# adi-gov-tw/Taiwan-Tongues-ASR-CE

Measured on AMD Instinct MI355X. Metric: audio-sec/s (RTF) whisper-large-v3 greedy, 30 s clips, batch 32; 1/2/4/8 GPU, higher is better.
Workload: dtype bf16; 1 GPU; whisper-large-v3 geometry (random-init seeded weights), 32 x 30 s 16 kHz synthetic clips per GPU in pinned host memory, H2D + log-mel + encoder + cross-KV + 4-token prompt + 128 greedy tokens (EOT suppressed), bf16; clips_per_gpu=32, contexts_per_gpu=1, parallelism=dp1

## Files before the change

taiwan_tongues_asr_ce_amd/csrc/common.hpp:

```cpp
#pragma once
#include <hip/hip_runtime.h>
#include <stdint.h>

typedef uint16_t bf16_t;

using f32x4 = __attribute__((ext_vector_type(4))) float;
using f32x16 = __attribute__((ext_vector_type(16))) float;
using s16x8 = __attribute__((ext_vector_type(8))) short;
using s16x4 = __attribute__((ext_vector_type(4))) short;

__device__ __forceinline__ float bf2f(bf16_t v) { return __uint_as_float(((uint32_t)v) << 16); }
__device__ __forceinline__ bf16_t f2bf(float f) { return __builtin_bit_cast(bf16_t, (__bf16)f); }
__device__ __forceinline__ uint32_t f2bf_pk(float lo, float hi) {
  typedef __bf16 bf16x2_hw __attribute__((ext_vector_type(2)));
  typedef float f32x2_hw __attribute__((ext_vector_type(2)));
  return __builtin_bit_cast(uint32_t, __builtin_convertvector((f32x2_hw){lo, hi}, bf16x2_hw));
}
struct f16_t { uint16_t bits; };
using h16x8 = __attribute__((ext_vector_type(8))) _Float16;
typedef _Float16 h16x2_hw __attribute__((ext_vector_type(2)));

template <typename T> struct N16;
template <> struct N16<bf16_t> {
  static __device__ __forceinline__ float up(uint16_t b) { return __uint_as_float(((uint32_t)b) << 16); }
// ... 90 lines not shown
  return v;
}
template <class T> __device__ __forceinline__ T* sgpr_pin_ptr(T* p) {
  typedef __attribute__((address_space(1))) T* global_ptr;
  global_ptr g = (global_ptr)p;
  asm volatile("" : "+s"(g));
  return (T*)g;
}


__device__ __forceinline__ int32_t sload_i32(const int32_t* p) {
  typedef const __attribute__((address_space(4))) int32_t* const_ptr;
  return *(const_ptr)p;
}
__device__ __forceinline__ int row_done_issue(const int32_t* done, int row, const void* valid) {
  return sload_i32(done ? done + row : (const int32_t*)valid);
}

struct GemmEpi {
  const float* bias = nullptr;
  int act = 0;
  const float* rowtab = nullptr;
  int rowmod = 0;
  const float* residual = nullptr;
  float* out_f32 = nullptr;
  void* out_t = nullptr;
  int64_t ldc = 0;
  int64_t batch_stride_c = 0;
  int headsplit = 0;
  int hs_T = 0, hs_H = 0, hs_d = 0;
  int64_t hs_which = 0;
};

struct GemmArgs {
  const void* A = nullptr;
  const void* W = nullptr;
  int M = 0, N = 0, K = 0;
  int64_t lda = 0, ldw = 0;
  int64_t batch_stride_a = 0;
  int batch = 1;
  int groups = 1;
  int64_t group_stride_w = 0, group_stride_out = 0;
  GemmEpi epi;
};

struct KernelOpts {
  int xattn_variant = 3;
  int xattn_deep_items = 512;
  int xattn_mq_slices = 0;
  int skinny_nt = 1;
  int skinny_narrow = 1;
  int skinny_x_lds = 1;
  int flash_qw = 2;
};

template <typename T> void launch_gemm_basic(const GemmArgs& g, hipStream_t s);
template <typename T16> void launch_gemm_bf16_fast(const GemmArgs& g, hipStream_t s);
bool gemm_bf16_fast_ok(const GemmArgs& g);
template <typename T16> void launch_gemm_bf16_v2(const GemmArgs& g, hipStream_t s);
bool gemm_bf16_v2_ok(const GemmArgs& g);
template <typename T16> void launch_gemm_bf16_v3(const GemmArgs& g, hipStream_t s);
bool gemm_bf16_v3_ok(const GemmArgs& g);
template <typename T16> void launch_gemm_bf16_v4(const GemmArgs& g, hipStream_t s);
bool gemm_bf16_v4_ok(const GemmArgs& g);
template <typename T16> bool launch_gemm_bf16_v5(const GemmArgs& g, hipStream_t s);
bool gemm_bf16_v5_ok(const GemmArgs& g);

template <typename T>
void launch_layernorm(const float* x, const float* gamma, const float* beta, T* out, int rows, int d, hipStream_t s);
template <typename T>
void launch_layernorm_add(float* x, const T* delta, const float* gamma, const float* beta, T* out, int rows, int d, hipStream_t s);
template <typename T>
void launch_layernorm_peek(const float* x, const T* delta, const float* gamma, const float* beta, T* out, int rows, int d, hipStream_t s);
template <typename T>
void launch_layernorm_add2(float* x, const T* delta, const T* delta2, const float* gamma, const float* beta, T* out, int rows, int d,
                           hipStream_t s);
struct LnPre {
  const float* bias = nullptr;
  const float* slab = nullptr;
  int n_slab = 0;
  int64_t slab_stride = 0;
  float* x_out = nullptr;
  const int32_t* tok = nullptr;
  const int32_t* step = nullptr;
  const void* emb = nullptr;
  const void* pos = nullptr;
};
template <typename T>
void launch_layernorm_rows(const float* x, const float* gamma, const float* beta, T* out, int rows, int d, const LnPre& pre,
                           hipStream_t s);
template <typename T>
void launch_layernorm_rows_embed_pos(const float* gamma, const float* beta, T* out, int rows, int d, const LnPre& pre, hipStream_t s);

struct SlabIn {
  const float* slab = nullptr;
  const float* bias = nullptr;
  int n = 0;
  int64_t stride = 0;
  int ld = 0;
};

template <typename T> struct RowVec;
template <> struct RowVec<float> {
  static constexpr int VEC = 4;
  __device__ static void load(const float* p, float (&v)[4]) {
    float4 t = *(const float4*)p;
// ... 2 lines not shown
};
template <typename T16> struct RowVec16 {
  static constexpr int VEC = 8;
  __device__ static void load(const T16* p, float (&v)[8]) {
    const uint4 t = *(const uint4*)p;
    up8<T16>(t, v);
  }
};
template <> struct RowVec<bf16_t> : RowVec16<bf16_t> {};
template <> struct RowVec<f16_t> : RowVec16<f16_t> {};

template <typename T>
__device__ __forceinline__ void load_row_slabs(const SlabIn& si, int64_t off, int col ,
                                               float (&v)[RowVec<T>::VEC]) {
  constexpr int VEC = RowVec<T>::VEC, NF4 = VEC / 4, MAXS = 4;
  float4 t[MAXS][NF4], bs[NF4];
#pragma unroll
  for (int c = 0; c < NF4; ++c) bs[c] = *(const float4*)(si.bias + col + 4 * c);
#pragma unroll
  for (int s = 0; s < MAXS; ++s) {
    const float* p = si.slab + (int64_t)min(s, si.n - 1) * si.stride + off;
#pragma unroll
    for (int c = 0; c < NF4; ++c) t[s][c] = *(const float4*)(p + 4 * c);
  }
  __builtin_amdgcn_sched_barrier(0);
#pragma unroll
  for (int c = 0; c < NF4; ++c) {
    float4 a = bs[c];
#pragma unroll
    for (int s = 0; s < MAXS; ++s)
      if (s == 0 || s < si.n) { a.x += t[s][c].x; a.y += t[s][c].y; a.z += t[s][c].z; a.w += t[s][c].w; }
    v[4 * c] = to_f<T>(from_f<T>(a.x)); v[4 * c + 1] = to_f<T>(from_f<T>(a.y));
    v[4 * c + 2] = to_f<T>(from_f<T>(a.z)); v[4 * c + 3] = to_f<T>(from_f<T>(a.w));
  }
}
struct QProj {
  const void* x = nullptr;
  const void* W = nullptr;
  const float* bias = nullptr;
};

template <typename T16> void launch_shuffle_cast(const float* src, T16* dst_base, int rows, int K, int row_offset, const KernelOpts& ko, hipStream_t s, int rows_total = 0);
int skinny_rows_per_block(int N, int K, const KernelOpts& ko);
template <typename T16>
bool launch_gemm_skinny(const T16* Wsh, const T16* x, int B, int N, int K, const GemmEpi& e, const KernelOpts& ko, hipStream_t s, int ksplit = 1,
                        float* slab = nullptr, int64_t slab_stride = 0);
int gemm_skinny_ksplit(int B, int N, int K, int want, const KernelOpts& ko);
template <typename T16> bool launch_gemm_vocab(const T16* Wsh, const T16* x, int B, int N, int K, float* out, int64_t ldc, const KernelOpts& ko, hipStream_t s, int device);
void gemm_vocab_init(int device);
void gemm_tiles_init(int device);
void launch_mel(const float* pcm, int64_t pcm_stride, const int64_t* n_samples_dev, int B, int n_mels, int n_frames,
                const float* filters , const float* dft_cos, const float* dft_sin ,
                const float* window , float* logmel , unsigned* clip_max ,
                hipStream_t s, const int64_t* geom_dev = nullptr);
unsigned mel_max_to_ordered(float v);
float mel_max_from_ordered(unsigned u);
template <typename T>
void launch_mel_finish(float* logmel, const unsigned* clip_max, T* mel_t , int B, int n_mels,
                       int n_frames, hipStream_t s, const int64_t* geom_dev = nullptr);
template <typename T>
void launch_mel_transpose(const float* mel, T* mel_t, int B, int n_mels, int n_frames, hipStream_t s);

template <typename T> void launch_enc_attn_simple(const T* qkv, T* out, int B, int T_, int H, hipStream_t s);
template <typename T16> void launch_enc_attn_flash_bf16(const T16* qkv, T16* out, int B, int T_, int H, const KernelOpts& ko, hipStream_t s);
template <typename T16>
void launch_cross_attn_flash_bf16(const T16* q, const T16* K, const T16* V, T16* out, int n_clips, int n_q, int H, int Tk, hipStream_t s);

struct RuleDyn { int32_t max_prompt, max_new, sot_index; uint32_t seed; };
struct DecState {
  int32_t* cur_tok;
  int32_t* step;
  int32_t* n_sampled;
  int32_t* last_tok;
  int32_t* pen_tok;
  int32_t* last_ts;
  int32_t* done;
  int32_t* n_done;
  float* sum_logprob;
  float* no_speech;
  int32_t* out_tokens;
  const int32_t* prompt;
  const int32_t* prompt_len;
  const uint8_t* mask;
  const RuleDyn* dyn;
  const int32_t* row_cap;
};
struct RuleParams {
  int V, ldv, max_prompt, max_new;
  int eot, no_timestamps, timestamp_begin, no_speech, sot_index, timestamps, max_initial, suppress_eot;
  float temperature;
  uint32_t seed;
};
template <typename T>
void launch_cross_attn_probs(const T* q, const T* K, const T* V, T* out, int rows, int H, int Tk, const int* sel ,
                             float* probs , hipStream_t s);
void launch_token_logprob(const float* logits, int ldv, int V, const int32_t* target, float* out, int rows, hipStream_t s);
void launch_token_prob(const float* logits, int ldv, int V, int tok, float* out , int rows, hipStream_t s);
template <typename T>
void launch_lang_head(const T* dh, const T* emb, int rows, int d, int V, int lang_begin, int n_lang, float* probs, int32_t* best,
                      float* logits, hipStream_t s);
struct LangRows {
  int32_t* pending; const int32_t* slot; int32_t* prompt; int max_prompt; int32_t* cur_tok; int32_t* row_pos;
  int32_t* best; float* probs; float* logits;
};
template <typename T>
void launch_lang_head_rows(const T* dh, const T* emb, int rows, int d, int V, int lang_begin, int n_lang, const LangRows& a, hipStream_t s);
void launch_lang_admit_rows(const int32_t* tab, int n, int B, int sot, int32_t* pending, int32_t* slot, int32_t* cur_tok, hipStream_t s);
// ... 74 lines not shown
```

taiwan_tongues_asr_ce_amd/csrc/engine.hip:

```cpp
#include "engine_ctx.hpp"
extern "C" {

const char* ttasr_version(void) { return "ttasr 0.4 (gfx950, HIP; f32 | bf16 | fp16)"; }

const char* ttasr_last_error(const ttasr_ctx* ctx) { return ctx ? ctx->err.c_str() : g_create_error.c_str(); }

static int create_impl(const ttasr_config* cfg, int device_id, ttasr_ctx* owner, ttasr_ctx** out_ctx);
static std::mutex g_share_mu;

int ttasr_create(const ttasr_config* cfg, int device_id, ttasr_ctx** out_ctx) {
  return guarded(nullptr, [&]() -> int { return create_impl(cfg, device_id, nullptr, out_ctx); });
}

int ttasr_create_shared(ttasr_ctx* owner, int32_t max_batch, ttasr_ctx** out_ctx) {
  return guarded(nullptr, [&]() -> int {
  if (!owner || !out_ctx) return fail(nullptr, TTASR_E_INVALID, "owner/out_ctx is NULL");
  *out_ctx = nullptr;
  if (owner->weight_owner) owner = owner->weight_owner;
  if (!owner->finalized) return fail(nullptr, TTASR_E_INVALID, "the owner's weights are not finalized (ttasr_finalize_weights first)");
  { std::lock_guard<std::mutex> lk(g_share_mu);
    if (owner->destroy_pending) return fail(nullptr, TTASR_E_INVALID, "the owner context was destroyed"); }
  ttasr_config cfg = owner->cfg;
  if (max_batch > 0) cfg.max_batch = max_batch;
  return create_impl(&cfg, owner->device, owner, out_ctx);
// ... 149 lines not shown

int ttasr_load_tensor_device(ttasr_ctx* c, const char* name, const void* data_dev, int32_t dtype, const int64_t* dims, int32_t ndim) {
  return guarded(c, [&]() -> int {
  if (!c) return TTASR_E_INVALID;
  TRY(weights_writable(c));
  if (!name || !data_dev || !dims) return fail(c, TTASR_E_INVALID, "NULL argument");
  if (dtype != TTASR_DTYPE_F32 && dtype != TTASR_DTYPE_BF16 && dtype != TTASR_DTYPE_F16)
    return fail(c, TTASR_E_INVALID, "dtype must be 0 (float32), 1 (bfloat16 bits) or 2 (float16 bits)");
  HIPCHK(c, hipSetDevice(c->device));
  return ingest_tensor(c, name, data_dev, dtype, dims, ndim);
  });
}

int ttasr_finalize_weights(ttasr_ctx* c) {
  return guarded(c, [&]() -> int {
  if (!c) return TTASR_E_INVALID;
  for (auto& kv : c->slots)
    if (!kv.second.loaded) return fail(c, TTASR_E_WEIGHTS, "tensor '%s' was never loaded", kv.first.c_str());
  c->finalized = true;
  return TTASR_OK;
  });
}

int ttasr_log_mel(ttasr_ctx* c, const float* pcm, int64_t pcm_stride, const int64_t* n_samples, int32_t B,
                  int32_t on_device, float* out_mel) {
  return guarded(c, [&]() -> int {
  if (!c) return TTASR_E_INVALID;
  TRY(session_refusal(c));
  if (B < 1 || B > c->maxB) return fail(c, TTASR_E_INVALID, "batch %d outside [1, %d]", B, c->maxB);
  if (!pcm || !n_samples) return fail(c, TTASR_E_INVALID, "pcm / n_samples is NULL");
  HIPCHK(c, hipSetDevice(c->device));
  hipStream_t s = c->stream;
  const float* src = pcm;
  int64_t stride = pcm_stride;
  std::vector<int64_t> ns(n_samples, n_samples + B);
  for (int b = 0; b < B; ++b) {
    if (ns[b] < 0 || ns[b] > pcm_stride) return fail(c, TTASR_E_INVALID, "n_samples[%d]=%lld outside [0, stride]", b, (long long)ns[b]);
    if (ns[b] > c->n_samples) ns[b] = c->n_samples;
  }
  hipEventRecord(c->ev[0], s);
  if (!on_device) {
    bool whole = pcm_stride == c->n_samples;
    for (int b = 0; b < B && whole; ++b) whole = ns[b] == c->n_samples;
    if (whole) {
      HIPCHK(c, hipMemcpyAsync(c->pcm_dev, pcm, (size_t)B * c->n_samples * 4, hipMemcpyHostToDevice, s));
    } else {
      for (int b = 0; b < B; ++b)
        if (ns[b] > 0)
          HIPCHK(c, hipMemcpyAsync(c->pcm_dev + (int64_t)b * c->n_samples, pcm + b * pcm_stride, ns[b] * 4, hipMemcpyHostToDevice, s));
    }
    src = c->pcm_dev; stride = c->n_samples;
  }
  HIPCHK(c, hipMemcpyAsync(c->nsamp_dev, ns.data(), B * 8, hipMemcpyHostToDevice, s));
  launch_mel(src, stride, c->nsamp_dev, B, c->M, c->F, c->filters, c->dcos, c->dsin, c->window, c->mel, c->clip_max, s);
  TT_DISPATCH(c, launch_mel_finish<T>(c->mel, c->clip_max, (T*)c->mel_t, B, c->M, c->F, s));
  hipEventRecord(c->ev[1], s);
  if (out_mel) HIPCHK(c, hipMemcpyAsync(out_mel, c->mel, (size_t)B * c->M * c->F * 4, hipMemcpyDeviceToHost, s));
  HIPCHK(c, hipStreamSynchronize(s));
  HIPCHK(c, hipGetLastError());
  hipEventElapsedTime(&c->phase_ms[0], c->ev[0], c->ev[1]);
  c->B_mel = B;
  return TTASR_OK;
  });
}

int ttasr_log_mel_windows(ttasr_ctx* c, const float* const* file_pcm_of, const int64_t* file_samples_of, const int64_t* seek_frames,
                          int32_t B, const float* floor_max, float* out_window_max, float* out_mel) {
  return guarded(c, [&]() -> int {
  if (!c) return TTASR_E_INVALID;
  TRY(session_refusal(c));
  if (B < 1 || B > c->maxB) return fail(c, TTASR_E_INVALID, "batch %d outside [1, %d]", B, c->maxB);
  if (!file_pcm_of || !file_samples_of || !seek_frames) return fail(c, TTASR_E_INVALID, "NULL argument");
  HIPCHK(c, hipSetDevice(c->device));
  hipStream_t s = c->stream;
  const int64_t stride = c->n_samples + 512;
  std::vector<int64_t> ns(B), geom((size_t)3 * B);
  hipEventRecord(c->ev[0], s);
  for (int b = 0; b < B; ++b) {
    const float* file_pcm = file_pcm_of[b];
    const int64_t file_samples = file_samples_of[b];
    if (!file_pcm || file_samples < 0) return fail(c, TTASR_E_INVALID, "window %d: recording is NULL / negative length", b);
    const int64_t file_frames = file_samples / 160;
    const int64_t seek = seek_frames[b];
    if (seek < 0 || seek > file_frames) return fail(c, TTASR_E_INVALID, "seek_frames[%d]=%lld outside the recording (%lld frames)", b, (long long)seek, (long long)file_frames);
    const WindowSpan w = window_span(c, file_samples, seek);
    ns[b] = w.n;
    memcpy(&geom[3 * (size_t)b], w.geom, sizeof w.geom);
    if (ns[b] > 0) HIPCHK(c, hipMemcpyAsync(c->pcm_dev + (int64_t)b * stride, file_pcm + w.first, ns[b] * 4, hipMemcpyHostToDevice, s));
  }
  HIPCHK(c, hipMemcpyAsync(c->nsamp_dev, ns.data(), B * 8, hipMemcpyHostToDevice, s));
  HIPCHK(c, hipMemcpyAsync(c->mel_geom, geom.data(), (size_t)B * 24, hipMemcpyHostToDevice, s));
  launch_mel(c->pcm_dev, stride, c->nsamp_dev, B, c->M, c->F, c->filters, c->dcos, c->dsin, c->window, c->mel, c->clip_max, s, c->mel_geom);
  std::vector<unsigned> mx(B);
  if (out_window_max) {
    HIPCHK(c, hipMemcpyAsync(mx.data(), c->clip_max, B * 4, hipMemcpyDeviceToHost, s));
    HIPCHK(c, hipStreamSynchronize(s));
    for (int b = 0; b < B; ++b) out_window_max[b] = mel_max_from_ordered(mx[b]);
  }
  if (floor_max) {
    for (int b = 0; b < B; ++b) mx[b] = mel_max_to_ordered(floor_max[b]);
    HIPCHK(c, hipMemcpyAsync(c->clip_max, mx.data(), B * 4, hipMemcpyHostToDevice, s));
  }
  TT_DISPATCH(c, launch_mel_finish<T>(c->mel, c->clip_max, (T*)c->mel_t, B, c->M, c->F, s, c->mel_geom));
  hipEventRecord(c->ev[1], s);
  if (out_mel) HIPCHK(c, hipMemcpyAsync(out_mel, c->mel, (size_t)B * c->M * c->F * 4, hipMemcpyDeviceToHost, s));
  HIPCHK(c, hipStreamSynchronize(s));
  HIPCHK(c, hipGetLastError());
  hipEventElapsedTime(&c->phase_ms[0], c->ev[0], c->ev[1]);
  c->B_mel = B;
  return TTASR_OK;
  });
}

int ttasr_set_mel(ttasr_ctx* c, const float* mel, int32_t B) {
  return guarded(c, [&]() -> int {
  if (!c) return TTASR_E_INVALID;
  TRY(session_refusal(c));
  if (B < 1 || B > c->maxB || !mel) return fail(c, TTASR_E_INVALID, "bad arguments");
  HIPCHK(c, hipSetDevice(c->device));
  HIPCHK(c, hipMemcpyAsync(c->mel, mel, (size_t)B * c->M * c->F * 4, hipMemcpyHostToDevice, c->stream));
  TT_DISPATCH(c, launch_mel_transpose<T>(c->mel, (T*)c->mel_t, B, c->M, c->F, c->stream));
  HIPCHK(c, hipStreamSynchronize(c->stream));
  HIPCHK(c, hipGetLastError());
  c->B_mel = B;
  return TTASR_OK;
  });
}

int ttasr_encode(ttasr_ctx* c, int32_t B, float* out_enc) {
  return guarded(c, [&]() -> int {
  TRY(check_ready(c, B));
  if (c->B_mel < B) return fail(c, TTASR_E_INVALID, "mel for %d clips requested but only %d resident", B, c->B_mel);
  sched_encoder(c, B);
  if (out_enc) {
    const int64_t n = (int64_t)B * c->T * c->d;
    if (c->lowp) { TT_DISPATCH(c, launch_uncast<T>((const T*)c->enc_out, c->x, n, c->stream));
                   HIPCHK(c, hipMemcpyAsync(out_enc, c->x, n * 4, hipMemcpyDeviceToHost, c->stream)); }
    else HIPCHK(c, hipMemcpyAsync(out_enc, c->enc_out, n * 4, hipMemcpyDeviceToHost, c->stream));
  }
  HIPCHK(c, hipStreamSynchronize(c->stream));
  HIPCHK(c, hipGetLastError());
  hipEventElapsedTime(&c->phase_ms[1], c->ev[2], c->ev[3]);
  hipEventElapsedTime(&c->phase_ms[2], c->ev[3], c->ev[4]);
  if (c->enc_timing) {
    for (float& v : c->enc_class_ms) v = 0.f;
// ... 806 lines not shown
```

taiwan_tongues_asr_ce_amd/csrc/engine_refill.hip:

```cpp
#include "engine_ctx.hpp"
#include <chrono>
#include <cmath>
#include <deque>

namespace ttasr_detail {

struct Session {
  struct Clip { int64_t id; std::vector<float> pcm; std::vector<int32_t> prompt; int32_t cap;
                bool win = false, has_floor = false; int64_t geom[3] = {0, 0, 0}; unsigned floor = 0;
                int mode = 0, rows = 0; float temp = 0.f; uint32_t seed = 0; int32_t sot = 0;
                int det = -1; };
  struct Lang { int idx = -1; std::vector<float> probs, logits; };
  struct Done { int64_t id; std::vector<int32_t> tok; float lp, ns; Lang lang; };
  ttasr_gen_opts o{};
  int max_prompt = 0;
  int64_t next_id = 0;
  std::deque<Clip> queue;
  std::vector<Clip> staged;
  size_t staged_next = 0;
  std::vector<int64_t> stage_ns;
  std::vector<int64_t> stage_geom;
  std::vector<unsigned> stage_floor;
  bool enc_pending = false;
  std::vector<int64_t> row_clip;
// ... 61 lines not shown

static int n_free_rows(const Session* S) {
  int n = 0;
  for (int64_t id : S->row_clip) n += id < 0;
  return n;
}

static int n_units(const ttasr_ctx* c, const Session* S) { return S->beam ? S->G : c->maxB; }
static int n_free_units(const Session* S) {
  if (!S->beam) return n_free_rows(S);
  int n = 0;
  for (const Session::Group& g : S->grp) n += g.clip < 0 && g.held < 0;
  return n;
}
static int n_held_units(const Session* S) {
  int n = 0;
  if (S->beam) { for (const Session::Group& g : S->grp) n += g.held >= 0; }
  else for (char h : S->held) n += h != 0;
  return n;
}

static int start_encode(ttasr_ctx* c, Session* S, int k) {
  hipStream_t es = S->es;
  S->staged.clear(); S->staged_next = 0;
  S->stage_ns.assign(k, 0);
  if (es != c->stream) HIPCHK(c, hipStreamWaitEvent(es, S->ev_copy, 0));
  HIPCHK(c, hipEventRecord(S->ev_enc0, es));
  bool any_win = false;
  for (int j = 0; j < k; ++j) {
    S->staged.push_back(std::move(S->queue.front()));
    S->queue.pop_front();
    any_win |= S->staged.back().win;
  }
  const int64_t stride = any_win ? c->n_samples + 512 : c->n_samples;
  S->stage_geom.assign(any_win ? 3 * (size_t)k : 0, 0);
  S->stage_floor.assign(k, 0);
  for (int j = 0; j < k; ++j) {
    const Session::Clip& cl = S->staged[j];
    S->stage_ns[j] = (int64_t)cl.pcm.size();
    if (any_win) {
      const int64_t plain[3] = {0, (int64_t)c->F * 160, c->F};
      memcpy(&S->stage_geom[3 * (size_t)j], cl.win ? cl.geom : plain, 24);
      if (!cl.win) S->stage_ns[j] = std::min<int64_t>(S->stage_ns[j], (int64_t)c->F * 160);
    }
    if (!cl.pcm.empty())
      HIPCHK(c, hipMemcpyAsync(c->pcm_dev + (int64_t)j * stride, cl.pcm.data(), cl.pcm.size() * 4, hipMemcpyHostToDevice, es));
  }
  HIPCHK(c, hipMemcpyAsync(c->nsamp_dev, S->stage_ns.data(), (size_t)k * 8, hipMemcpyHostToDevice, es));
  const int64_t* geom = nullptr;
  if (any_win) {
    HIPCHK(c, hipMemcpyAsync(c->mel_geom, S->stage_geom.data(), (size_t)k * 24, hipMemcpyHostToDevice, es));
    geom = c->mel_geom;
  }
  launch_mel(c->pcm_dev, stride, c->nsamp_dev, k, c->M, c->F, c->filters, c->dcos, c->dsin, c->window, c->mel, c->clip_max, es, geom);
  for (int j = 0; j < k; ++j) {
    const Session::Clip& cl = S->staged[j];
    if (!cl.has_floor) continue;
    S->stage_floor[j] = cl.floor;
    HIPCHK(c, hipMemcpyAsync(c->clip_max + j, &S->stage_floor[j], 4, hipMemcpyHostToDevice, es));
  }
  TT_DISPATCH(c, launch_mel_finish<T>(c->mel, c->clip_max, (T*)c->mel_t, k, c->M, c->F, es, geom));
  void* const xkv = c->xkv;
  const int gemm_force = c->gemm_force;
  if (gemm_force == 0) c->gemm_force = 3;
  c->xkv = c->xkv_stage; c->cur = es;
  sched_encoder(c, k);
  c->xkv = xkv; c->cur = c->stream; c->gemm_force = gemm_force;
  HIPCHK(c, hipEventRecord(S->ev_enc, es));
  S->enc_pending = es != c->stream;
  S->encodes++; S->clips_encoded += k;
  return 0;
}

static int flush_quant_pairs(ttasr_ctx* c, const XkvSlotPairs& qp, int& n) {
  if (n == 0) return 0;
  TT_DISPATCH(c, launch_xkv_quant_slots<T>((const T*)c->xkv_stage, c->xkv8, c->xkv8_scale, c->cfg.dec_layers, c->H, c->T, c->maxB,
                                           c->xkv_which_elems, qp, n, c->stream));
  n = 0;
  HIPCHK(c, hipGetLastError());
  return 0;
}

static int prefill_collect(ttasr_ctx* c, Session* S) {
  if (!S->pf_busy) return 0;
  HIPCHK(c, hipEventSynchronize(S->ev_pf));
  for (size_t i = 0; i + 1 < S->pf_ev_used; i += 2) {
    float ms = 0.f;
    if (hipEventElapsedTime(&ms, S->pf_ev[i], S->pf_ev[i + 1]) == hipSuccess) S->pf_ms += ms;
  }
  S->pf_ev_used = 0; S->pf_busy = false;
  return 0;
}

static int run_prefill_passes(ttasr_ctx* c, Session* S, const std::vector<PrefillSeq>& sq) {
  if (sq.empty()) return 0;
  TRY(prefill_collect(c, S));
  hipStream_t s = c->stream;
  const int pps = c->pages_per_seq;
  std::vector<int> len(sq.size());
  for (size_t i = 0; i < sq.size(); ++i) len[i] = sq[i].len;
  const std::vector<int> cut = prefill_pass_split(len, kPrefillRowCap);
  std::vector<PrefillPass> passes;
  size_t w = 0;
  for (size_t k = 0; k + 1 < cut.size(); ++k) {
    int rows = 0, items = 0;
    const int n = cut[k + 1] - cut[k];
    for (int i = cut[k]; i < cut[k + 1]; ++i) { rows += len[i]; items += prefill_items_of(len[i]); }
// ... 899 lines not shown
```

taiwan_tongues_asr_ce_amd/csrc/engine_search.hip:

```cpp
#include "engine_ctx.hpp"
#include <chrono>

namespace ttasr_detail {

int check_ready(ttasr_ctx* c, int B) {
  if (!c) return TTASR_E_INVALID;
  if (!c->finalized) return fail(c, TTASR_E_INVALID, "weights not finalized (call ttasr_finalize_weights first)");
  TRY(session_refusal(c));
  if (B < 1 || B > c->maxB) return fail(c, TTASR_E_INVALID, "batch %d outside [1, max_batch=%d]", B, c->maxB);
  HIPCHK(c, hipSetDevice(c->device));
  return 0;
}

int upload_rules(ttasr_ctx* c, const ttasr_gen_opts* o, int max_prompt) {
  if (!o) return fail(c, TTASR_E_INVALID, "opts is NULL");
  if (o->max_new_tokens < 1 || o->max_new_tokens > c->max_new_alloc)
    return fail(c, TTASR_E_INVALID, "max_new_tokens %d outside [1, %d]", o->max_new_tokens, c->max_new_alloc);
  std::vector<uint8_t> mask(c->V, 0);
  for (int i = 0; i < o->n_suppress; ++i) {
    int t = o->suppress[i];
    if (t < 0 || t >= c->V) return fail(c, TTASR_E_INVALID, "suppress id %d outside vocabulary", t);
    mask[t] |= 1;
  }
  for (int i = 0; i < o->n_begin_suppress; ++i) {
// ... 36 lines not shown
  if (key == "ingest_chunk") {
    if (v < 0 || v > 1 << 30) return 1;
    c->ingest_chunk = v;
    return 0;
  }
  if (key == "wire_chunk") {
    if (v < 0 || v > 1 << 30) return 1;
    c->wire_chunk = v;
    return 0;
  }
  if (key == "seg_lstm_rows") {
    if (v != 0 && v != 1 && v != 2 && v != 4) return 1;
    c->seg_lstm_rows = v;
    return 0;
  }
  if (key == "ingest_timing") { c->ingest_timing = on; return 0; }
  if (key == "flash") c->no_flash = !on;
  else if (key == "prefill") c->no_prefill = !on;
  else if (key == "vocab_persistent") c->vocab_persistent = on;
  else if (key == "xsplit") c->no_xsplit = !on;
  else if (key == "graph") c->use_graph = on;
  else if (key == "multi_step_graph") c->multi_step = on;
  else if (key == "generic_kernels") c->force_basic = on;
  else if (key == "prefill_tiled") c->prefill_tiled = on;
  else if (key == "prefill_ns_min") { if (v < 0) return 1; c->prefill_ns_min = v; }
  else if (key == "enc_residual_epilogue") c->enc_res_epilogue = on;
  else if (key == "enc_gemm") { if (v < 0 || v > 4) return 1; c->gemm_force = v; }
  else if (key == "enc_gemm_persistent") c->gemm_persistent = on;
  else if (key == "xkv_grouped") c->xkv_grouped = on;
  else if (key == "enc_gemm_tail") c->gemm_tail = on;
  else if (key == "enc_ln_defer") c->enc_ln_defer = on;
  else if (key == "dec_narrow_blocks") { if (c->weights_packed && on != (c->ko.skinny_narrow != 0)) return 1; c->ko.skinny_narrow = on; }
  else if (key == "ksplit_out") { if (v < 0 || v > 16) return 1; c->ks_want[0] = v; }
  else if (key == "ksplit_q") { if (v < 0 || v > 16) return 1; c->ks_want[1] = v; }
  else if (key == "ksplit_qkv") { if (v < 0 || v > 16) return 1; c->ks_want[2] = v; }
  else if (key == "ksplit_fc2") { if (v < 0 || v > 16) return 1; c->ks_want[3] = v; }
  else if (key == "xattn_nontemporal") c->ko.xattn_variant = (c->ko.xattn_variant & ~1) | (on ? 1 : 0);
  else if (key == "xattn_pipeline") c->ko.xattn_variant = (c->ko.xattn_variant & ~2) | (on ? 2 : 0);
  else if (key == "xkv_fp8") {
    if (v < 0 || v > 2) return 1;
    if (on && !c->lowp) return 1;
    if (on && (!c->xkv8 || !c->xkv8_scale)) {
      const size_t n = (size_t)c->cfg.dec_layers * c->xkv_layer_elems;
      if (!c->xkv8_scale && dalloc(c, &c->xkv8_scale, (size_t)c->cfg.dec_layers * 2 * c->maxB * c->H * sizeof(float)) != 0) return 2;
      if (!c->xkv8 && dalloc(c, &c->xkv8, n, false) != 0) return 2;
    }
    c->xkv_fp8 = v; c->xkv8_valid = false;
  }
  else if (key == "xattn_mq_fp8") c->xattn_mq_fp8 = on;
  else if (key == "weights_nontemporal") c->ko.skinny_nt = on;
  else if (key == "dec_x_lds") c->ko.skinny_x_lds = on;
  else if (key == "ragged_exit") c->ragged_exit = on;
  else if (key == "flash_qw") { if (v < 1 || v > 2) return 1; c->ko.flash_qw = v; }
  else if (key == "xattn_mq_slices") { if (v < 0 || v > 8) return 1; c->ko.xattn_mq_slices = v; }
  else if (key == "xattn_deep_items") { if (v < 0 || v > 1 << 20) return 1; c->ko.xattn_deep_items = v; }
  else return 1;
  drop_graphs(c);
  return 0;
}

int reset_search(ttasr_ctx* c, int B) {
  hipStream_t s = c->stream;
  HIPCHK(c, hipMemsetAsync(c->st.step, 0, 16, s));
  HIPCHK(c, hipMemsetAsync(c->st.n_sampled, 0, B * 4, s));
  HIPCHK(c, hipMemsetAsync(c->st.last_tok, 0xff, B * 4, s));
  HIPCHK(c, hipMemsetAsync(c->st.pen_tok, 0xff, B * 4, s));
  HIPCHK(c, hipMemsetAsync(c->st.last_ts, 0xff, B * 4, s));
  HIPCHK(c, hipMemsetAsync(c->st.done, 0, B * 4, s));
  HIPCHK(c, hipMemsetAsync(c->st.n_done, 0, 16, s));
  HIPCHK(c, hipMemsetAsync(c->st.sum_logprob, 0, B * 4, s));
  HIPCHK(c, hipMemsetAsync(c->st.no_speech, 0, B * 4, s));
  HIPCHK(c, hipMemsetAsync(c->row_cap_dev, 0x7f, B * 4, s));
  return 0;
}

int check_prompt(ttasr_ctx* c, int i, const int32_t* row, int len, int max_prompt, const int32_t* sot) {
  if (len < 1 || len > max_prompt) return fail(c, TTASR_E_INVALID, "prompt %d: length %d outside [1, %d]", i, len, max_prompt);
  if (len >= c->cfg.n_text_ctx)
    return fail(c, TTASR_E_INVALID, "prompt %d: length %d leaves no room in the %d-token context", i, len, c->cfg.n_text_ctx);
  for (int j = 0; j < len; ++j)
    if (row[j] < 0 || row[j] >= c->V) return fail(c, TTASR_E_INVALID, "prompt %d: token %d at %d outside the vocabulary", i, row[j], j);
  if (sot && (*sot < 0 || *sot >= len)) return fail(c, TTASR_E_INVALID, "prompt %d: sot_index %d outside the %d-token prompt", i, *sot, len);
  return 0;
}

int generate_rows(ttasr_ctx* c, int R, int rows_per_clip, const int32_t* prompt, const int32_t* prompt_len, int max_prompt,
                  const ttasr_gen_opts* o, float temperature, uint32_t seed, int32_t* out_tokens, int32_t* out_len, float* out_lp,
                  float* out_ns, const int32_t* row_cap) {
  int min_plen = 1 << 30, max_plen = 0;
  const int A = R / rows_per_clip;
  for (int a = 0; a < A; ++a) {
    TRY(check_prompt(c, a, prompt + (size_t)a * max_prompt, prompt_len[a], max_prompt, nullptr));
    min_plen = std::min(min_plen, prompt_len[a]); max_plen = std::max(max_plen, prompt_len[a]);
  }
  int max_cap = o->max_new_tokens;
  if (row_cap) {
    max_cap = 1;
    for (int r = 0; r < R; ++r) {
      if (row_cap[r] < 1 || row_cap[r] > o->max_new_tokens)
        return fail(c, TTASR_E_INVALID, "row_max_new[%d]=%d outside [1, max_new_tokens=%d]", r, row_cap[r], o->max_new_tokens);
      max_cap = std::max(max_cap, (int)row_cap[r]);
    }
  }
  SearchScope scope(c, StepShape{rows_per_clip, 1, false}, c->prompt_dev, c->plen_dev, R);
  RuleParams old = c->rp;
  TRY(upload_rules(c, o, max_prompt));
// ... 294 lines not shown
```

taiwan_tongues_asr_ce_amd/csrc/kernels_misc.hip:

```cpp
#include "common.hpp"
#include <cstring>

__device__ __forceinline__ unsigned f2ord(float f) {
  unsigned u = __float_as_uint(f);
  return (u & 0x80000000u) ? ~u : (u | 0x80000000u);
}
__device__ __forceinline__ float ord2f(unsigned u) {
  return __uint_as_float((u & 0x80000000u) ? (u & 0x7fffffffu) : ~u);
}

constexpr int MEL_F = 8;
constexpr int MEL_SPAN = 160 * (MEL_F - 1) + 400;

__global__ __launch_bounds__(256) void mel_kernel(const float* __restrict__ pcm, int64_t pcm_stride,
                                                  const int64_t* __restrict__ n_samples, int n_mels, int n_frames,
                                                  const float* __restrict__ filters, const float* __restrict__ dcos,
                                                  const float* __restrict__ dsin, const float* __restrict__ window,
                                                  float* __restrict__ logmel, unsigned* __restrict__ clip_max,
                                                  const int64_t* __restrict__ geom) {
  __shared__ float xs[MEL_SPAN];
  __shared__ float tc[400], tsn[400], win[400];
  __shared__ float pw[MEL_F][208];
  __shared__ float red[4];
  const int b = blockIdx.y, f0 = blockIdx.x * MEL_F, tid = threadIdx.x;
  const int64_t lead = geom ? geom[3 * b] : 0;
  const int64_t total = geom ? geom[3 * b + 1] : (int64_t)n_frames * 160;
  const int valid_frames = geom ? (int)geom[3 * b + 2] : n_frames;
  const int64_t n_valid = geom ? n_samples[b] : min((int64_t)n_frames * 160, n_samples[b]);
  const float* x = pcm + (int64_t)b * pcm_stride;
  for (int i = tid; i < 400; i += 256) { tc[i] = dcos[i]; tsn[i] = dsin[i]; win[i] = window[i]; }
  for (int i = tid; i < MEL_SPAN; i += 256) {
    int64_t sidx = lead + (int64_t)f0 * 160 - 200 + i;
    if (sidx < 0) sidx = -sidx;
    if (sidx >= total) sidx = 2 * (total - 1) - sidx;
    xs[i] = (sidx >= 0 && sidx < n_valid) ? x[sidx] : 0.0f;
  }
  __syncthreads();
  if (tid < 201) {
    float re[MEL_F], im[MEL_F];
#pragma unroll
    for (int f = 0; f < MEL_F; ++f) { re[f] = 0.f; im[f] = 0.f; }
    int idx = 0;
    for (int n = 0; n < 400; ++n) {
      float c = tc[idx], s = tsn[idx], w = win[n];
#pragma unroll
      for (int f = 0; f < MEL_F; ++f) {
        float v = xs[f * 160 + n] * w;
        re[f] = fmaf(v, c, re[f]);
        im[f] = fmaf(v, s, im[f]);
      }
      idx += tid;
      if (idx >= 400) idx -= 400;
    }
#pragma unroll
    for (int f = 0; f < MEL_F; ++f) pw[f][tid] = re[f] * re[f] + im[f] * im[f];
  }
  __syncthreads();
  float lmax = -1e30f;
  for (int o = tid; o < n_mels * MEL_F; o += 256) {
    int m = o % n_mels, f = o / n_mels;
    if (f0 + f < n_frames) {
      float acc = 0.f;
      for (int k = 0; k < 201; ++k) acc = fmaf(pw[f][k], filters[k * n_mels + m], acc);
      float l = log10f(fmaxf(acc, 1e-10f));
      logmel[((int64_t)b * n_mels + m) * n_frames + f0 + f] = l;
      if (f0 + f < valid_frames) lmax = fmaxf(lmax, l);
    }
  }
  lmax = wave_max(lmax);
  if ((tid & 63) == 0) red[tid >> 6] = lmax;
  __syncthreads();
  if (tid == 0) atomicMax(&clip_max[b], f2ord(fmaxf(fmaxf(red[0], red[1]), fmaxf(red[2], red[3]))));
}

void launch_mel(const float* pcm, int64_t pcm_stride, const int64_t* n_samples_dev, int B, int n_mels, int n_frames,
                const float* filters, const float* dft_cos, const float* dft_sin, const float* window, float* logmel,
                unsigned* clip_max, hipStream_t s, const int64_t* geom_dev) {
  hipMemsetAsync(clip_max, 0, sizeof(unsigned) * B, s);
  dim3 grid((n_frames + MEL_F - 1) / MEL_F, B);
  hipLaunchKernelGGL(mel_kernel, grid, dim3(256), 0, s, pcm, pcm_stride, n_samples_dev, n_mels, n_frames, filters,
                     dft_cos, dft_sin, window, logmel, clip_max, geom_dev);
}
unsigned mel_max_to_ordered(float v) { unsigned u; memcpy(&u, &v, 4); return (u & 0x80000000u) ? ~u : (u | 0x80000000u); }
float mel_max_from_ordered(unsigned u) { u = (u & 0x80000000u) ? (u & 0x7fffffffu) : ~u; float v; memcpy(&v, &u, 4); return v; }

template <typename T>
__global__ __launch_bounds__(256) void mel_finish_kernel(float* __restrict__ logmel, const unsigned* __restrict__ clip_max,
                                                         T* __restrict__ mel_t, int n_mels, int n_frames, int normalise,
                                                         const int64_t* __restrict__ geom) {
  __shared__ float tile[32][33];
  const int b = blockIdx.z, f0 = blockIdx.x * 32, m0 = blockIdx.y * 32;
  const int tx = threadIdx.x & 31, ty = threadIdx.x >> 5;
  const float floor_v = normalise ? ord2f(clip_max[b]) - 8.0f : 0.f;
  const int valid_frames = geom ? (int)geom[3 * b + 2] : n_frames;
  for (int r = ty; r < 32; r += 8) {
    int m = m0 + r, f = f0 + tx;
    if (m < n_mels && f < n_frames) {
      int64_t i = ((int64_t)b * n_mels + m) * n_frames + f;
      float v = logmel[i];
      if (normalise) {
        v = f < valid_frames ? (fmaxf(v, floor_v) + 4.0f) * 0.25f : 0.f;
        logmel[i] = v;
      }
      tile[r][tx] = v;
    }
  }
  __syncthreads();
  for (int r = ty; r < 32; r += 8) {
    int f = f0 + r, m = m0 + tx;
    if (m < n_mels && f < n_frames) mel_t[((int64_t)b * (n_frames + 2) + f + 1) * n_mels + m] = from_f<T>(tile[tx][r]);
  }
  if (blockIdx.x == 0 && blockIdx.y == 0) {
    for (int i = threadIdx.x; i < n_mels; i += 256) {
      mel_t[(int64_t)b * (n_frames + 2) * n_mels + i] = from_f<T>(0.f);
      mel_t[((int64_t)b * (n_frames + 2) + n_frames + 1) * n_mels + i] = from_f<T>(0.f);
    }
  }
}

template <typename T>
void launch_mel_finish(float* logmel, const unsigned* clip_max, T* mel_t, int B, int n_mels, int n_frames, hipStream_t s,
                       const int64_t* geom_dev) {
  dim3 grid((n_frames + 31) / 32, (n_mels + 31) / 32, B);
  hipLaunchKernelGGL(mel_finish_kernel<T>, grid, dim3(256), 0, s, logmel, clip_max, mel_t, n_mels, n_frames, 1, geom_dev);
}
template <typename T>
void launch_mel_transpose(const float* mel, T* mel_t, int B, int n_mels, int n_frames, hipStream_t s) {
  dim3 grid((n_frames + 31) / 32, (n_mels + 31) / 32, B);
  hipLaunchKernelGGL(mel_finish_kernel<T>, grid, dim3(256), 0, s, (float*)mel, (const unsigned*)nullptr, mel_t, n_mels,
                     n_frames, 0, (const int64_t*)nullptr);
}
// ... 299 lines not shown
```

Baseline: 2232 audio-s/s.

## Add register-blocked mel spectrogram kernel with 64-frame tiles and reused twiddles

Adds a new mel kernel, enabled by default through a new mel_form option. Each block handles 64 frames, with each wave computing 16 frames across 4 frequency bins per lane in registers. Twiddles are packed as float2 in LDS and indexed modularly, so each cos/sin load is shared across 16 frames. The mel filterbank pass then reads 8 frames per thread with vector LDS loads and vector stores. This is meant to cut redundant twiddle and filter loads in the DFT and filterbank stages, at the cost of heavy register pressure and fewer blocks. Mel is a small share of the end-to-end pipeline.

Result: no change. 2234 audio-s/s (median of 6 runs) (+0.1%).

```diff
diff --git a/taiwan_tongues_asr_ce_amd/csrc/common.hpp b/taiwan_tongues_asr_ce_amd/csrc/common.hpp
--- a/taiwan_tongues_asr_ce_amd/csrc/common.hpp
+++ b/taiwan_tongues_asr_ce_amd/csrc/common.hpp
@@ -166,6 +166,7 @@
   int skinny_narrow = 1;
   int skinny_x_lds = 1;
   int flash_qw = 2;
+  int mel_form = 1;
 };
 
 template <typename T> void launch_gemm_basic(const GemmArgs& g, hipStream_t s);
@@ -274,7 +275,7 @@
 void launch_mel(const float* pcm, int64_t pcm_stride, const int64_t* n_samples_dev, int B, int n_mels, int n_frames,
                 const float* filters , const float* dft_cos, const float* dft_sin ,
                 const float* window , float* logmel , unsigned* clip_max ,
-                hipStream_t s, const int64_t* geom_dev = nullptr);
+                const KernelOpts& ko, hipStream_t s, const int64_t* geom_dev = nullptr);
 unsigned mel_max_to_ordered(float v);
 float mel_max_from_ordered(unsigned u);
 template <typename T>
diff --git a/taiwan_tongues_asr_ce_amd/csrc/engine.hip b/taiwan_tongues_asr_ce_amd/csrc/engine.hip
--- a/taiwan_tongues_asr_ce_amd/csrc/engine.hip
+++ b/taiwan_tongues_asr_ce_amd/csrc/engine.hip
@@ -225,7 +225,7 @@
     src = c->pcm_dev; stride = c->n_samples;
   }
   HIPCHK(c, hipMemcpyAsync(c->nsamp_dev, ns.data(), B * 8, hipMemcpyHostToDevice, s));
-  launch_mel(src, stride, c->nsamp_dev, B, c->M, c->F, c->filters, c->dcos, c->dsin, c->window, c->mel, c->clip_max, s);
+  launch_mel(src, stride, c->nsamp_dev, B, c->M, c->F, c->filters, c->dcos, c->dsin, c->window, c->mel, c->clip_max, c->ko, s);
   TT_DISPATCH(c, launch_mel_finish<T>(c->mel, c->clip_max, (T*)c->mel_t, B, c->M, c->F, s));
   hipEventRecord(c->ev[1], s);
   if (out_mel) HIPCHK(c, hipMemcpyAsync(out_mel, c->mel, (size_t)B * c->M * c->F * 4, hipMemcpyDeviceToHost, s));
@@ -263,7 +263,7 @@
   }
   HIPCHK(c, hipMemcpyAsync(c->nsamp_dev, ns.data(), B * 8, hipMemcpyHostToDevice, s));
   HIPCHK(c, hipMemcpyAsync(c->mel_geom, geom.data(), (size_t)B * 24, hipMemcpyHostToDevice, s));
-  launch_mel(c->pcm_dev, stride, c->nsamp_dev, B, c->M, c->F, c->filters, c->dcos, c->dsin, c->window, c->mel, c->clip_max, s, c->mel_geom);
+  launch_mel(c->pcm_dev, stride, c->nsamp_dev, B, c->M, c->F, c->filters, c->dcos, c->dsin, c->window, c->mel, c->clip_max, c->ko, s, c->mel_geom);
   std::vector<unsigned> mx(B);
   if (out_window_max) {
     HIPCHK(c, hipMemcpyAsync(mx.data(), c->clip_max, B * 4, hipMemcpyDeviceToHost, s));
diff --git a/taiwan_tongues_asr_ce_amd/csrc/engine_refill.hip b/taiwan_tongues_asr_ce_amd/csrc/engine_refill.hip
--- a/taiwan_tongues_asr_ce_amd/csrc/engine_refill.hip
+++ b/taiwan_tongues_asr_ce_amd/csrc/engine_refill.hip
@@ -137,7 +137,7 @@
     HIPCHK(c, hipMemcpyAsync(c->mel_geom, S->stage_geom.data(), (size_t)k * 24, hipMemcpyHostToDevice, es));
     geom = c->mel_geom;
   }
-  launch_mel(c->pcm_dev, stride, c->nsamp_dev, k, c->M, c->F, c->filters, c->dcos, c->dsin, c->window, c->mel, c->clip_max, es, geom);
+  launch_mel(c->pcm_dev, stride, c->nsamp_dev, k, c->M, c->F, c->filters, c->dcos, c->dsin, c->window, c->mel, c->clip_max, c->ko, es, geom);
   for (int j = 0; j < k; ++j) {
     const Session::Clip& cl = S->staged[j];
     if (!cl.has_floor) continue;
diff --git a/taiwan_tongues_asr_ce_amd/csrc/engine_search.hip b/taiwan_tongues_asr_ce_amd/csrc/engine_search.hip
--- a/taiwan_tongues_asr_ce_amd/csrc/engine_search.hip
+++ b/taiwan_tongues_asr_ce_amd/csrc/engine_search.hip
@@ -112,6 +112,7 @@
   else if (key == "dec_x_lds") c->ko.skinny_x_lds = on;
   else if (key == "ragged_exit") c->ragged_exit = on;
   else if (key == "flash_qw") { if (v < 1 || v > 2) return 1; c->ko.flash_qw = v; }
+  else if (key == "mel_form") c->ko.mel_form = on;
   else if (key == "xattn_mq_slices") { if (v < 0 || v > 8) return 1; c->ko.xattn_mq_slices = v; }
   else if (key == "xattn_deep_items") { if (v < 0 || v > 1 << 20) return 1; c->ko.xattn_deep_items = v; }
   else return 1;
diff --git a/taiwan_tongues_asr_ce_amd/csrc/kernels_misc.hip b/taiwan_tongues_asr_ce_amd/csrc/kernels_misc.hip
--- a/taiwan_tongues_asr_ce_amd/csrc/kernels_misc.hip
+++ b/taiwan_tongues_asr_ce_amd/csrc/kernels_misc.hip
@@ -73,10 +73,128 @@
   if (tid == 0) atomicMax(&clip_max[b], f2ord(fmaxf(fmaxf(red[0], red[1]), fmaxf(red[2], red[3]))));
 }
 
+constexpr int MEL_FW = 16;
+__global__ __launch_bounds__(256, 2) void mel_rb_kernel(const float* __restrict__ pcm, int64_t pcm_stride,
+                                                  const int64_t* __restrict__ n_samples, int n_mels, int n_frames,
+                                                  const float* __restrict__ filters, const float* __restrict__ dcos,
+                                                  const float* __restrict__ dsin, const float* __restrict__ window,
+                                                  float* __restrict__ logmel, unsigned* __restrict__ clip_max,
+                                                  const int64_t* __restrict__ geom) {
+  constexpr int FW = MEL_FW, WF = 4 * FW;
+  constexpr int SPAN = 160 * (WF - 1) + 400;
+  constexpr int PWS = WF + 4;
+  constexpr int REGION = SPAN > 201 * PWS ? SPAN : 201 * PWS;
+  __shared__ __attribute__((aligned(16))) float buf[REGION];
+  __shared__ __attribute__((aligned(16))) float2 tw[400];
+  __shared__ __attribute__((aligned(16))) float win[400];
+  __shared__ float red[4];
+  float* xs = buf;
+  float* pw = buf;
+  const int b = blockIdx.y, f0 = blockIdx.x * WF, tid = threadIdx.x, lane = tid & 63, wave = tid >> 6;
+  const int64_t lead = geom ? geom[3 * b] : 0;
+  const int64_t total = geom ? geom[3 * b + 1] : (int64_t)n_frames * 160;
+  const int valid_frames = geom ? (int)geom[3 * b + 2] : n_frames;
+  const int64_t n_valid = geom ? n_samples[b] : min((int64_t)n_frames * 160, n_samples[b]);
+  const float* x = pcm + (int64_t)b * pcm_stride;
+  for (int i = tid; i < 400; i += 256) { tw[i] = make_float2(dcos[i], dsin[i]); win[i] = window[i]; }
+  for (int i = tid; i < SPAN; i += 256) {
+    int64_t sidx = lead + (int64_t)f0 * 160 - 200 + i;
+    if (sidx < 0) sidx = -sidx;
+    if (sidx >= total) sidx = 2 * (total - 1) - sidx;
+    xs[i] = (sidx >= 0 && sidx < n_valid) ? x[sidx] : 0.0f;
+  }
+  __syncthreads();
+  typedef float f32x2 __attribute__((ext_vector_type(2)));
+  f32x2 acc[4][FW];
+#pragma unroll
+  for (int j = 0; j < 4; ++j)
+#pragma unroll
+    for (int f = 0; f < FW; ++f) acc[j][f] = f32x2{0.f, 0.f};
+  {
+    const float* xw = xs + wave * (FW * 160);
+    unsigned idx[4] = {0u, 0u, 0u, 0u};
+#pragma unroll 1
+    for (int n = 0; n < 400; n += 2) {
+      const float2 w2 = *(const float2*)(win + n);
+      float v[FW][2];
+#pragma unroll
+      for (int f = 0; f < FW; ++f) {
+        const float2 x2 = *(const float2*)(xw + f * 160 + n);
+        v[f][0] = x2.x * w2.x; v[f][1] = x2.y * w2.y;
+      }
+#pragma unroll
+      for (int t = 0; t < 2; ++t)
+#pragma unroll
+        for (int j = 0; j < 4; ++j) {
+          const f32x2 cs = *(const f32x2*)((const char*)tw + idx[j]);
+#pragma unroll
+          for (int f = 0; f < FW; ++f) acc[j][f] = __builtin_elementwise_fma(f32x2{v[f][t], v[f][t]}, cs, acc[j][f]);
+          idx[j] += 8u * (unsigned)(lane + 64 * j);
+          idx[j] = min(idx[j], idx[j] - 3200u);
+        }
+    }
+  }
+  __syncthreads();
+#pragma unroll
+  for (int j = 0; j < 4; ++j) {
+    const int k = lane + 64 * j;
+    if (k < 201) {
+#pragma unroll
+      for (int f = 0; f < FW; f += 4) {
+        float p[4];
+#pragma unroll
+        for (int i = 0; i < 4; ++i) p[i] = fmaf(acc[j][f + i].x, acc[j][f + i].x, acc[j][f + i].y * acc[j][f + i].y);
+        *(float4*)(pw + k * PWS + wave * FW + f) = make_float4(p[0], p[1], p[2], p[3]);
+      }
+    }
+  }
+  __syncthreads();
+  float lmax = -1e30f;
+  for (int o = tid; o < n_mels * (WF / 8); o += 256) {
+    const int m = o % n_mels, fb = f0 + (o / n_mels) * 8;
+    if (fb >= n_frames) continue;
+    const float* pr = pw + (fb - f0);
+    float acc[8];
+#pragma unroll
+    for (int i = 0; i < 8; ++i) acc[i] = 0.f;
+#pragma unroll 3
+    for (int k = 0; k < 201; ++k) {
+      const float w = filters[k * n_mels + m];
+      const float4 p0 = *(const float4*)(pr + k * PWS), p1 = *(const float4*)(pr + k * PWS + 4);
+      acc[0] = fmaf(p0.x, w, acc[0]); acc[1] = fmaf(p0.y, w, acc[1]); acc[2] = fmaf(p0.z, w, acc[2]); acc[3] = fmaf(p0.w, w, acc[3]);
+      acc[4] = fmaf(p1.x, w, acc[4]); acc[5] = fmaf(p1.y, w, acc[5]); acc[6] = fmaf(p1.z, w, acc[6]); acc[7] = fmaf(p1.w, w, acc[7]);
+    }
+    float l[8];
+#pragma unroll
+    for (int i = 0; i < 8; ++i) {
+      l[i] = log10f(fmaxf(acc[i], 1e-10f));
+      if (fb + i < n_frames && fb + i < valid_frames) lmax = fmaxf(lmax, l[i]);
+    }
+    float* dst = logmel + ((int64_t)b * n_mels + m) * n_frames + fb;
+    if ((n_frames & 3) == 0 && fb + 8 <= n_frames) {
+      *(float4*)dst = make_float4(l[0], l[1], l[2], l[3]);
+      *(float4*)(dst + 4) = make_float4(l[4], l[5], l[6], l[7]);
+    } else {
+#pragma unroll
+      for (int i = 0; i < 8; ++i)
+        if (fb + i < n_frames) dst[i] = l[i];
+    }
+  }
+  lmax = wave_max(lmax);
+  if (lane == 0) red[wave] = lmax;
+  __syncthreads();
+  if (tid == 0) atomicMax(&clip_max[b], f2ord(fmaxf(fmaxf(red[0], red[1]), fmaxf(red[2], red[3]))));
+}
+
 void launch_mel(const float* pcm, int64_t pcm_stride, const int64_t* n_samples_dev, int B, int n_mels, int n_frames,
                 const float* filters, const float* dft_cos, const float* dft_sin, const float* window, float* logmel,
-                unsigned* clip_max, hipStream_t s, const int64_t* geom_dev) {
+                unsigned* clip_max, const KernelOpts& ko, hipStream_t s, const int64_t* geom_dev) {
   hipMemsetAsync(clip_max, 0, sizeof(unsigned) * B, s);
+  if (ko.mel_form) {
+    hipLaunchKernelGGL(mel_rb_kernel, dim3((n_frames + 4 * MEL_FW - 1) / (4 * MEL_FW), B), dim3(256), 0, s, pcm, pcm_stride,
+                       n_samples_dev, n_mels, n_frames, filters, dft_cos, dft_sin, window, logmel, clip_max, geom_dev);
+    return;
+  }
   dim3 grid((n_frames + MEL_F - 1) / MEL_F, B);
   hipLaunchKernelGGL(mel_kernel, grid, dim3(256), 0, s, pcm, pcm_stride, n_samples_dev, n_mels, n_frames, filters,
                      dft_cos, dft_sin, window, logmel, clip_max, geom_dev);
```
